# biaslab/GaussianProcessNode

Measured on AMD Instinct MI355X. Metric: VMP iterations/sec (sparse-GP node sweep, kin40k-shaped synthetic), higher is better.
Workload: dtype f64

## Files before the change

gaussianprocessnode_amd/csrc/sgp_api.hip:

```cpp
#include "../../include/sgp_hip.h"
#include "sgp_kernels.hip.h"

#include <algorithm>
#include <atomic>
#include <chrono>
#include <cmath>
#include <cstdio>
#include <cstdlib>
#include <dlfcn.h>
#include <cstring>
#include <limits>
#include <mutex>
#include <string>
#include <type_traits>
#include <vector>

using namespace sgp;

namespace {

thread_local std::string g_create_error;
std::atomic<int> g_live_handles{0};

std::mutex g_registry_mutex;
// ... 276 lines not shown
    SyrkGeom g;
    g.row_lo = row_lo;
    g.nrows = nrows;
    g.tile0 = row_lo * (row_lo + 1) / 2;
    g.ntiles = (row_lo + nrows) * (row_lo + nrows + 1) / 2 - g.tile0;
    g.chunk = wide ? 4 * SYRK_WAVES : KB;
    g.nchunks = 0;
    g.wide = wide ? 1 : 0;
    if (n <= 0) return g;
    if (wide) {
        const int want = std::max(1, std::max(8, cus) / g.ntiles);
        int64_t per = (n + want - 1) / want;
        per = std::max<int64_t>(4 * SYRK_WAVES, (per + 4 * SYRK_WAVES - 1) / (4 * SYRK_WAVES) * (4 * SYRK_WAVES));
        g.chunk = (int)per;
        g.nchunks = (int)std::max<int64_t>(1, (n + per - 1) / per);
        return g;
    }
    const int slots = SYRK_BLOCKS_PER_CU * std::max(8, cus);
    int a = 8;
    for (int q = 2; q <= 8; q *= 2)
        if (g.ntiles % q == 0) a = 8 / q;
    int want = std::max(1, slots / g.ntiles);
    if (want > a) want = want / a * a;
    int64_t per = (n + want - 1) / want;
    per = std::max<int64_t>(KB, (per + KB - 1) / KB * KB);
    g.chunk = (int)per;
    g.nchunks = (int)std::max<int64_t>(1, (n + per - 1) / per);
    if (g.nchunks > a) g.nchunks = (g.nchunks + a - 1) / a * a;
    return g;
}
static inline size_t syrk_items(const SyrkGeom& g) { return (size_t)g.ntiles * g.nchunks; }
static inline unsigned assemble_z(const SyrkGeom& g) { return g.nchunks <= 24 ? 4u : 16u; }
static void launch_syrk(const SyrkGeom& g, hipStream_t s, const double* Kuf, const double* omega, double* slabs, int Mp, int64_t n,
                        int64_t* stamps, long long* gate, long long gate_value) {
    if (g.wide)
        hipLaunchKernelGGL(k_syrk_direct, dim3((unsigned)((syrk_items(g) + 7) / 8 * 8)), dim3(SYRK_DIRECT_THREADS), 0, s, Kuf, omega, slabs, Mp, n,
                           g, stamps, gate, gate_value);
    else
        hipLaunchKernelGGL(k_syrk_stream, dim3((unsigned)syrk_items(g)), dim3(256), 0, s, Kuf, omega, slabs, Mp, n, g, stamps, gate,
                           gate_value);
}

struct PotrfSeq {
    double* A; int ld, Tn; int* info; int n_valid; double* scratch; hipStream_t s;
    double* Winv; LamForm form; bool has_form; double* Sacc; const double* tv_xi; double* tv_t; const hipEvent_t* step_wait;
    int j = 0;
    PotrfSeq(double* A_, int ld_, int Tn_, int* info_, int n_valid_, double* scratch_, hipStream_t s_, double* Winv_ = nullptr,
             const LamForm* form_ = nullptr, double* Sacc_ = nullptr, const double* tv_xi_ = nullptr, double* tv_t_ = nullptr,
             const hipEvent_t* step_wait_ = nullptr)
        : A(A_), ld(ld_), Tn(Tn_), info(info_), n_valid(n_valid_), scratch(scratch_), s(s_), Winv(Winv_), has_form(form_ != nullptr),
          Sacc(Sacc_), tv_xi(tv_xi_), tv_t(tv_t_), step_wait(step_wait_) {
        if (form_) form = *form_;
        else { memset(&form, 0, sizeof form); }
    }
    int extras(int jj) const {
        if (!Winv) return 0;
        int e = 0;
        if (jj >= 2) {
            e += 2 * (jj - 1) * (jj < Tn ? 2 : 1);
            if (Sacc && jj < Tn) e += (jj - 1) * jj / 2;
        }
        if (tv_t && jj >= 1) e += 1;
        return e;
    }
    bool done() const { return j > Tn; }
    void next() {
        LamForm none;
        memset(&none, 0, sizeof none);
        none.trace_chain = has_form ? 1 : 0;
        if (j < Tn) {
            const int nt = Tn - j;
            if (step_wait && step_wait[j]) (void)hipStreamWaitEvent(s, step_wait[j], 0);
            hipLaunchKernelGGL(k_potrf_step, dim3(nt * (nt + 1) / 2 + potrf_twins(Tn, j) + extras(j)), dim3(PSTEP_THREADS), 0, s, A, ld, j, Tn, info,
                               n_valid, scratch, Winv, Sacc, tv_xi, tv_t, has_form ? form : none);
        } else if (j == Tn && Winv && extras(Tn) > 0) {
            hipLaunchKernelGGL(k_potrf_step, dim3(extras(Tn)), dim3(PSTEP_THREADS), 0, s, A, ld, Tn, Tn, info, n_valid, scratch, Winv, Sacc,
                               tv_xi, tv_t, none);
        }
        ++j;
    }
};
static void launch_potrf(double* A, int ld, int Tn, int* info, int n_valid, double* scratch, hipStream_t s,
                         double* Winv = nullptr, const LamForm* form = nullptr, double* Sacc = nullptr,
                         const double* tv_xi = nullptr, double* tv_t = nullptr, const hipEvent_t* step_wait = nullptr) {
    PotrfSeq q(A, ld, Tn, info, n_valid, scratch, s, Winv, form, Sacc, tv_xi, tv_t, step_wait);
    while (!q.done()) q.next();
}

static void launch_ata(const double* W, double* C, int ld, int Tn, hipStream_t s, int rev = 0, const double* mu = nullptr,
                       double* R = nullptr, const double* Psi2 = nullptr, const double* Kinv = nullptr,
                       double* trace_part = nullptr, const UvArgs* uv = nullptr, const double* Sacc = nullptr) {
    const int extra = uv ? Tn * Tn : 0;
    hipLaunchKernelGGL(k_gemm32, dim3(Tn * (Tn + 1) / 2 * 4 + extra), dim3(256), 0, s, W, W, C, ld, Tn, 0, 0, rev, mu, R, Psi2,
                       Kinv, trace_part, uv ? *uv : UvArgs{}, Sacc);
}
static void launch_gemm(const double* A, const double* B, double* C, int ld, int Tn, hipStream_t s) {
    hipLaunchKernelGGL(k_gemm32, dim3(Tn * Tn * 4), dim3(256), 0, s, A, B, C, ld, Tn, 3, 0, 0, (const double*)nullptr, (double*)nullptr,
                       (const double*)nullptr, (const double*)nullptr, (double*)nullptr, UvArgs{}, (const double*)nullptr);
}


extern "C" int sgp_abi_version(void) { return SGP_ABI_VERSION; }

extern "C" const char* sgp_last_error(const sgp_handle* h) { return h ? h->err.c_str() : g_create_error.c_str(); }

template <typename T>
static hipError_t dalloc(T** p, size_t count) {
    *p = nullptr;
    if (count == 0) count = 1;
    return hipMalloc(reinterpret_cast<void**>(p), count * sizeof(T));
}

extern "C" int sgp_create(const sgp_config* cfg, sgp_handle** out) {
    if (!cfg || !out) return fail(nullptr, SGP_ERR_ARG, "sgp_create: null argument");
    *out = nullptr;
    if (cfg->m < 1 || cfg->d < 1 || cfg->d > MAXD || cfg->d_out < 1 || cfg->d_out > MAXO || cfg->n_max < 1)
        return fail(nullptr, SGP_ERR_ARG, "sgp_create: need m >= 1, 1 <= d <= 32, 1 <= d_out <= 4, n_max >= 1");
    if ((int64_t)cfg->m * cfg->d_out > CU_MAXQ - TB)
        return fail(nullptr, SGP_ERR_ARG, "sgp_create: d_out * m is limited to 4032 in this build");
    int ndev = 0;
    if (hipGetDeviceCount(&ndev) != hipSuccess || ndev == 0)
        return fail(nullptr, SGP_ERR_NODEVICE, "sgp_create: no HIP device visible (the HIP path has no CPU fallback)");
    if (cfg->device < 0 || cfg->device >= ndev) return fail(nullptr, SGP_ERR_ARG, "sgp_create: bad device ordinal");
    HIPCHK((sgp_handle*)nullptr, hipSetDevice(cfg->device));
    hipDeviceProp_t prop;
    HIPCHK((sgp_handle*)nullptr, hipGetDeviceProperties(&prop, cfg->device));
    if (strncmp(prop.gcnArchName, "gfx950", 6) != 0)
        return fail(nullptr, SGP_ERR_NODEVICE, "sgp_create: device is not gfx950 (MI355X); this library is built for gfx950 only");
// ... 595 lines not shown
    prep_main(h, s, h->n <= 0);
    if (h->n > 0) {
        launch_gram(h, s, true);
        long long* gate = h->gate_side ? h->dJoin + WORD_GATE : nullptr;
        launch_syrk(h->geom, s, h->dKuf, omega_of(h), h->dSlabs, Mp, h->n, h->dStamps + STAMP_STRIDE * SGP_T_SYRK, gate, h->gate_epoch);
    }
    SyrkGeom ga = h->geom;
    if (h->n <= 0) { ga = syrk_geometry(0, T, h->num_cus, 0); }
    hipLaunchKernelGGL(k_assemble, dim3(T, T + 1, assemble_z(ga)), dim3(256), 0, s, h->dSlabs, h->dBpart, h->dDataScal,
                       pack ? h->dPack : h->dStats, Mp, T, ga, h->n > 0 ? h->nblk : 0, h->dout,
                       SGP_S_COUNT + h->dout * h->dout, 1, h->dStamps + STAMP_STRIDE * SGP_T_LOCAL, h->dInfo + 1, (long long*)nullptr, 0LL,
                       pack ? 1 : 0, h->dBred);
}

static int exchange_stats(sgp_handle* h, hipStream_t s, int tile0, int ntile, bool with_tail);
static int enqueue_stats_overlapped(sgp_handle* h, const SweepPlan& p) {
    const int Mp = h->Mp, T = h->T;
    hipStream_t own = p.stream;
    const bool sharded = p.pack;
    prep_main(h, own, h->n <= 0);
    if (h->n > 0) launch_gram(h, own, true);
    hipLaunchKernelGGL(k_join_wait, dim3(1), dim3(64), 0, h->statM, (const long long*)(h->dJoin + WORD_ASM0), h->stat_epoch,
                       h->spin_limit, h->dInfo + 3, (int)SYNC_LATE_COLUMN, 8);
    for (int g = 0; g < h->ngroups; ++g) {
        const StatGroup& G = h->grp[g];
        hipStream_t s = G.masked ? h->statM : own;
        if (h->n > 0)
            launch_syrk(G.geom, s, h->dKuf, omega_of(h), h->dSlabs + G.slab_off, Mp, h->n,
                        h->dStamps + STAMP_STRIDE * SGP_T_SYRK, g == 0 ? h->dJoin + WORD_GATE : (long long*)nullptr, h->gate_epoch);
        hipLaunchKernelGGL(k_assemble, dim3(G.nrows, T + (g == 0 ? 1 : 0), assemble_z(G.geom)), dim3(256), 0, s, h->dSlabs + G.slab_off, h->dBpart,
                           h->dDataScal, sharded ? h->dPack : h->dStats, Mp, T, G.geom, h->nblk, h->dout,
                           SGP_S_COUNT + h->dout * h->dout, g == 0 ? 1 : 0, h->dStamps + STAMP_STRIDE * SGP_T_LOCAL,
                           g == 0 ? h->dInfo + 1 : (int*)nullptr, g == 0 ? h->dJoin + WORD_ASM0 : (long long*)nullptr, h->stat_epoch,
                           sharded ? 1 : 0, h->dBred);
        if (sharded) {
            if (int xrc = exchange_stats(h, s, G.geom.tile0, G.geom.ntiles, g == 0)) return xrc;
            if (G.masked && hipEventRecord(h->evGroup[g], s) != hipSuccess) return fail(h, SGP_ERR_HIP, "hipEventRecord failed (statistics group)");
        } else if (G.masked)
            hipLaunchKernelGGL(k_join_set, dim3(1), dim3(64), 0, s, h->dJoin + WORD_GROUP0 + g, h->stat_epoch);
    }
    return 0;
}

static void enqueue_finish1(sgp_handle* h, hipStream_t s, const SweepPlan& p) {
    const int M = h->M, Mp = h->Mp, Q = h->Q, Qp = h->Qp, TQ = h->TQ;
    LamForm form;
    memset(&form, 0, sizeof form);
    form.stats = h->dStats; form.Lambda0 = h->dLambda0; form.xi0 = h->dXi0; form.xi = h->dXi; form.P = h->dParams;
    form.M = M; form.Mp = Mp; form.d_out = h->dout; form.Q = Q; form.prior_form = h->prior_form;
    form.stamps = h->dStamps + STAMP_STRIDE * SGP_T_FINISH1;
    form.spin_limit = h->spin_limit;
    form.sync_status = h->dInfo + 3;
    form.trace_chain = 1;
    hipEvent_t step_wait[LAM_MAX_COLS] = {nullptr};
    bool any_wait = false;
    if (p.overlapped) {
        form.col_words = h->dJoin + WORD_GROUP0;
        form.col_need = h->stat_epoch;
        for (int g = 0; g < h->ngroups; ++g) {
            for (int c = h->grp[g].c0; c < h->grp[g].c1; ++c) {
                form.form_step[c] = (unsigned char)h->grp[g].form_step;
                form.col_group[c] = (h->grp[g].masked && !p.pack && !p.resident) ? (unsigned char)g : (unsigned char)0xff;
            }
            if (h->grp[g].masked && p.pack && !p.resident) { step_wait[h->grp[g].form_step] = h->evGroup[g]; any_wait = true; }
        }
    }
    double* uvt0 = h->dUvWork + 2 * (size_t)Qp;
    PotrfSeq lam(h->dLam, Qp, TQ, h->dInfo + 1, Qp, h->dScratch + POTRF_SCRATCH, s, h->dWl, &form, h->dTmp, h->dXi, uvt0,
                 any_wait ? step_wait : nullptr);
    if (p.kuu_interleaved) {
        PotrfSeq kuu(h->dKuu, h->Mp, h->T, h->dInfo + 0, h->M, h->dScratch, h->side, h->dWk, nullptr, h->dSaccK);
        while (!lam.done() || !kuu.done()) {
            if (!lam.done()) lam.next();
            if (!kuu.done()) kuu.next();
        }
        kuu_tail(h, h->side, p.join_word);
    } else {
        while (!lam.done()) lam.next();
    }
    double* uvp = h->dXi;
    double* uvck = h->dUvWork;
    double* uvak = h->dUvWork + Qp;
    double* uvt = uvt0;
    double* uvpart = uvt + (size_t)TQ * Qp;
    hipLaunchKernelGGL(k_trmv_mu_scan, dim3(Qp / 4 + 1 + TQ * (TQ + 1) / 2), dim3(256), 0, s, (const double*)h->dWl,
                       (const double*)uvt, h->dMu, uvp, uvck, uvak, uvpart, Qp);
}

static double* mirror_for(const sgp_handle* h) {
    return (h->hMirror && !h->env_no_zero_copy && !h->training) ? h->hMirror : nullptr;
}

static void launch_traces(sgp_handle* h, hipStream_t s) {
    hipLaunchKernelGGL(k_trace_kinv, dim3(TRACE_BLOCKS), dim3(256), 0, s, h->dStats, h->dKinv, h->dTrace, h->M, h->Mp);
    hipLaunchKernelGGL(k_trace_R, dim3(TRACE_BLOCKS), dim3(256), 0, s, h->dStats, h->dR, h->dTrace + TRACE_BLOCKS, h->M, h->Mp, h->dout,
                       h->Qp, (int64_t*)nullptr);
}

static void enqueue_finish2(sgp_handle* h, hipStream_t s, bool join_word) {
    const int M = h->M, Mp = h->Mp, Q = h->Q, Qp = h->Qp, TQ = h->TQ;
    double* uvp = h->dXi;
    double* uvck = h->dUvWork;
    double* uvak = h->dUvWork + Qp;
    double* uvpart = h->dUvWork + 2 * (size_t)Qp + (size_t)TQ * Qp;
    const int nata = TQ * (TQ + 1) / 2 * 4;
    double* traceR = h->dTrace + TRACE_BLOCKS;
    const double* partK = h->dTrace;
    int nK = TRACE_BLOCKS, nR = TRACE_BLOCKS;
    UvArgs uv;
    uv.Wp = h->dWl; uv.p = uvp; uv.ck = uvck; uv.ak = uvak; uv.partial = uvpart; uv.LR = h->dUvT;
    uv.stamps = h->dStamps + STAMP_STRIDE * SGP_T_FINISH1;
    uv.join = join_word ? h->dJoin + WORD_JOIN : nullptr;
    uv.join_need = h->join_epoch;
    uv.spin_limit = h->spin_limit;
    uv.sync_status = h->dInfo + 3;
    if (h->dout == 1) {
        launch_ata(h->dWl, h->dSigma, Qp, TQ, s, 1, h->dMu, h->dR, h->dStats, h->dKinv, traceR, &uv, h->dTmp);
        partK = traceR + nata;
        nK = nR = nata;
    } else {
        launch_ata(h->dWl, h->dSigma, Qp, TQ, s, 1, h->dMu, h->dR, nullptr, nullptr, nullptr, &uv, h->dTmp);
        launch_traces(h, s);
    }
    hipLaunchKernelGGL(k_scalars, dim3(1), dim3(256), 0, s, h->dStats, partK, nK, (const double*)traceR, nR, h->dMu, h->dKuu,
                       h->dLam, h->dInfo, h->dParams, h->dOut, h->dWishart, M, Mp, h->dout, Q, Qp, Qp - Q,
                       h->dStamps + STAMP_STRIDE * SGP_T_FINISH2, h->dStamps, h->dStampTotals,
                       h->dJoin + WORD_DONE, h->done_epoch,
                       (const double*)(h->dScratch + POTRF_LOGDET), h->T, (const double*)(h->dScratch + POTRF_SCRATCH + POTRF_LOGDET), TQ,
                       mirror_for(h));
}

static int set_device_checked(int device) {
    int ndev = 0;
    if (hipGetDeviceCount(&ndev) != hipSuccess || ndev == 0) return fail(nullptr, SGP_ERR_NODEVICE, "no HIP device visible");
    if (device < 0 || device >= ndev) return fail(nullptr, SGP_ERR_ARG, "bad device ordinal");
    if (hipSetDevice(device) != hipSuccess) return fail(nullptr, SGP_ERR_HIP, "hipSetDevice failed");
    return 0;
}

// ... 1162 lines not shown
```

gaussianprocessnode_amd/csrc/sgp_kernels.hip.h:

```cpp
#pragma once
#include <hip/hip_runtime.h>
#include <stdint.h>
#include <utility>

namespace sgp {

constexpr int TB = 64;
constexpr int PS = 80;
constexpr int KB = 16;
constexpr int MAXD = 32;
constexpr int MAXO = 4;
constexpr int LT = TB + 1;

typedef double d4 __attribute__((ext_vector_type(4)));

struct Params {
    double sigma2;
    double jitter;
    double E_logw;
    double n_override;
    double inv_ell[MAXD];
    double W[MAXO * MAXO];
    double prior_iso;
    double pad[7];
// ... 1144 lines not shown
            acc = __builtin_amdgcn_mfma_f64_16x16x4f64(Wt[(rb + li) * LT + rb + 4 * s4 + lk], Tw[(4 * s4 + lk) * 17 + li],
                                                       acc, 0, 0, 0);
#pragma unroll
        for (int r = 0; r < 4; ++r) Wt[(rb + lk + 4 * r) * LT + cb + li] = -acc[r];
    }
    __syncthreads();
    {
        const int ti = wave >> 1, tj = wave & 1;
        d4 acc = (d4){0.0, 0.0, 0.0, 0.0};
#pragma unroll
        for (int s4 = 0; s4 < 8; ++s4)
            acc = __builtin_amdgcn_mfma_f64_16x16x4f64(S[(32 + 16 * ti + li) * LT + 4 * s4 + lk],
                                                       Wt[(4 * s4 + lk) * LT + 16 * tj + li], acc, 0, 0, 0);
#pragma unroll
        for (int r = 0; r < 4; ++r) T[(16 * ti + lk + 4 * r) * 33 + 16 * tj + li] = acc[r];
        __syncthreads();
        acc = (d4){0.0, 0.0, 0.0, 0.0};
#pragma unroll
        for (int s4 = 0; s4 < 8; ++s4)
            acc = __builtin_amdgcn_mfma_f64_16x16x4f64(Wt[(32 + 16 * ti + li) * LT + 32 + 4 * s4 + lk],
                                                       T[(4 * s4 + lk) * 33 + 16 * tj + li], acc, 0, 0, 0);
#pragma unroll
        for (int r = 0; r < 4; ++r) Wt[(32 + 16 * ti + lk + 4 * r) * LT + 16 * tj + li] = -acc[r];
    }
    __syncthreads();
}

struct TileRegs { double v[16]; };
__device__ __forceinline__ void tile_g2r(TileRegs& t, const double* __restrict__ A, size_t ld, int row0, int col0) {
#pragma unroll
    for (int u = 0; u < 8; ++u) {
        const int e = (threadIdx.x & 255) + 256 * u, c = e >> 5, r = (e & 31) * 2;
        const double2 w = *reinterpret_cast<const double2*>(A + (size_t)(col0 + c) * ld + row0 + r);
        t.v[2 * u] = w.x;
        t.v[2 * u + 1] = w.y;
    }
}
constexpr int LAM_MAX_GROUPS = 8;
constexpr int LAM_MAX_COLS = 64;
struct LamForm {
    const double* stats;
    const double* Lambda0;
    const double* xi0;
    double* xi;
    const Params* P;
    int M, Mp, d_out, Q, prior_form;
    int64_t* stamps;
    const long long* col_words;
    long long col_need;
    unsigned char form_step[LAM_MAX_COLS], col_group[LAM_MAX_COLS];
    int spin_limit;
    int* sync_status;
    int trace_chain;
};
__device__ __forceinline__ double load_agent(const double* p) {
    return __hip_atomic_load((const __attribute__((address_space(1))) double*)p, __ATOMIC_RELAXED, __HIP_MEMORY_SCOPE_AGENT);
}
template <bool DENSE, bool MULTI, bool BYPASS = false>
__device__ __forceinline__ double lambda_entry(const LamForm& f, int gi, int gj, int Qp, double prior_iso, double w00) {
    const bool inside = gi < f.Q && gj < f.Q;
    const int si = inside ? gi : 0, sj = inside ? gj : 0;
    int a = 0, i = si, b = 0, j = sj;
    if constexpr (MULTI) { a = si / f.M; i = si % f.M; b = sj / f.M; j = sj % f.M; }
    double psi;
    if constexpr (BYPASS) psi = load_agent(f.stats + (size_t)j * f.Mp + i); else psi = f.stats[(size_t)j * f.Mp + i];
    const double diag = (gi == gj) ? 1.0 : 0.0;
    double prior, w;
    if constexpr (DENSE) prior = f.Lambda0[(size_t)sj * Qp + si]; else prior = diag * prior_iso;
    if constexpr (MULTI) w = f.P->W[a + b * f.d_out]; else w = w00;
    const double m = inside ? 1.0 : 0.0;
    return fma(m * w, psi, fma(m, prior, (1.0 - m) * diag));
}
template <bool DENSE, bool MULTI, bool BYPASS>
__device__ __forceinline__ void tile_form_r_impl(TileRegs& t, const LamForm& f, int Qp, int row0, int col0) {
    const double prior_iso = BYPASS ? load_agent(&f.P->prior_iso) : f.P->prior_iso, w00 = BYPASS ? load_agent(&f.P->W[0]) : f.P->W[0];
#pragma unroll
    for (int u = 0; u < 16; ++u) {
        const int e = (threadIdx.x & 255) + 256 * (u >> 1), c = e >> 5, r = (e & 31) * 2 + (u & 1);
        t.v[u] = lambda_entry<DENSE, MULTI, BYPASS>(f, Qp - 1 - (row0 + r), Qp - 1 - (col0 + c), Qp, prior_iso, w00);
    }
}
__device__ __forceinline__ void tile_form_r(TileRegs& t, const LamForm& f, int Qp, int row0, int col0, bool bypass = false) {
    const bool dense = f.prior_form == 1, multi = f.d_out > 1;
    if (bypass && !multi) {
        if (dense) tile_form_r_impl<true, false, true>(t, f, Qp, row0, col0); else tile_form_r_impl<false, false, true>(t, f, Qp, row0, col0);
        return;
    }
    if (dense) { if (multi) tile_form_r_impl<true, true, false>(t, f, Qp, row0, col0); else tile_form_r_impl<true, false, false>(t, f, Qp, row0, col0); }
    else       { if (multi) tile_form_r_impl<false, true, false>(t, f, Qp, row0, col0); else tile_form_r_impl<false, false, false>(t, f, Qp, row0, col0); }
}
__device__ __forceinline__ void tile_r2s(double* S, const TileRegs& t) {
#pragma unroll
    for (int u = 0; u < 16; ++u) {
        const int e = (threadIdx.x & 255) + 256 * (u >> 1), c = e >> 5, r = (e & 31) * 2 + (u & 1);
        S[r * LT + c] = t.v[u];
    }
}
__device__ __forceinline__ void tile_g2s(double* S, const double* __restrict__ A, size_t ld, int row0, int col0) {
    TileRegs t;
    tile_g2r(t, A, ld, row0, col0);
    tile_r2s(S, t);
}
__device__ __forceinline__ void tile_fetch(TileRegs& t, bool do_form, bool load_old, const double* __restrict__ A, const LamForm& f,
                                           int ld, int row0, int col0, bool bypass) {
    if (do_form) {
        tile_form_r(t, f, ld, row0, col0, bypass);
// ... 211 lines not shown
            const int row = wave * 16 + lk + 4 * r;
            Bs[row * PS32 + li] = t0a[r] + t0b[r];
            Bs[row * PS32 + 16 + li] = t1a[r] + t1b[r];
        }
        __syncthreads();
        d4 o0a = Z, o1a = Z, o0b = Z, o1b = Z;
        winv_half_mma(o0a, o1a, o0b, o1b, As, Bs, lane, wave);
        __syncthreads();
#pragma unroll
        for (int r = 0; r < 4; ++r) { o0[r] = -(o0a[r] + o0b[r]); o1[r] = -(o1a[r] + o1b[r]); }
    }
#pragma unroll
    for (int r = 0; r < 4; ++r) {
        const int row = wave * 16 + lk + 4 * r;
        Os[li * LT + row] = o0[r];
        Os[(16 + li) * LT + row] = o1[r];
    }
    __syncthreads();
    for (int e = tid; e < 32 * TB; e += 256) {
        const int jj = e >> 6, r = e & 63;
        W[(size_t)(col0 + jj) * ld + i * TB + r] = Os[jj * LT + r];
    }
}

__device__ __forceinline__ void sigma_row_tile(const double* __restrict__ W, double* __restrict__ Sacc, int ld, int i, int I,
                                               int J, double* panels, double* tile) {
    const int tid = threadIdx.x, lane = tid & 63, wave = tid >> 6, wr = wave >> 1, wc = wave & 1;
    double* As = panels;
    double* Bs = panels + TB * PS;
    load_panel_t(As, W, ld, i * TB, I * TB, TB, tid);
    if (I != J) load_panel_t(Bs, W, ld, i * TB, J * TB, TB, tid);
    if (I == i) {
        for (int e = tid; e < TB * LT; e += 256) tile[e] = 0.0;
    } else {
        tile_g2s(tile, Sacc, ld, I * TB, J * TB);
    }
    __syncthreads();
    Acc4 acc;
    acc_zero(acc);
    tile_mma(acc, As, (I != J) ? Bs : As, TB, lane, wr, wc);
#pragma unroll
    for (int ti = 0; ti < 2; ++ti)
#pragma unroll
        for (int tj = 0; tj < 2; ++tj)
#pragma unroll
            for (int r = 0; r < 4; ++r) acc.t[ti][tj][r] = -acc.t[ti][tj][r];
    tile_sub_acc(tile, acc, lane, wr, wc);
    __syncthreads();
    tile_s2g(tile, Sacc, ld, I * TB, J * TB);
}

template <int NP>
__device__ __forceinline__ void tvec_role(const double* __restrict__ L, const double* __restrict__ W,
                                          const double* __restrict__ xi, double* __restrict__ t, int ld, int i, double* lds) {
    constexpr int CP = TB / NP;
    double* red = lds;
    double* rvec = lds + NP * TB;
    const int tid = threadIdx.x, r = tid & 63, part = tid >> 6;
    const double* wb = W + (size_t)(i * TB + CP * part) * ld + i * TB + r;
    double wv[CP];
#pragma unroll
    for (int u = 0; u < CP; ++u) wv[u] = wb[(size_t)u * ld];
    double acc = 0.0;
    for (int k = 0; k < i; k += 4) {
        double v[4][CP], tv[4][CP];
#pragma unroll
        for (int q = 0; q < 4; ++q) {
            const int kq = (k + q < i) ? k + q : i - 1;
            const double live = (k + q < i) ? 1.0 : 0.0;
            const double* base = L + (size_t)(kq * TB + CP * part) * ld + i * TB + r;
#pragma unroll
            for (int u = 0; u < CP; ++u) { v[q][u] = base[(size_t)u * ld]; tv[q][u] = t[kq * TB + CP * part + u] * live; }
        }
#pragma unroll
        for (int q = 0; q < 4; ++q)
#pragma unroll
            for (int u = 0; u < CP; ++u) acc = fma(v[q][u], tv[q][u], acc);
    }
    auto tree = [&](int row) {
        double a[NP];
#pragma unroll
        for (int q = 0; q < NP; ++q) a[q] = red[q * TB + row];
#pragma unroll
        for (int w = 1; w < NP; w <<= 1)
#pragma unroll
            for (int q = 0; q + w < NP; q += 2 * w) a[q] += a[q + w];
        return a[0];
    };
    red[part * TB + r] = acc;
    __syncthreads();
    if (part == 0) rvec[r] = xi[ld - 1 - (i * TB + r)] - tree(r);
    __syncthreads();
    double s = 0.0;
#pragma unroll
    for (int u = 0; u < CP; ++u) s = fma(wv[u], rvec[CP * part + u], s);
    __syncthreads();
    red[part * TB + r] = s;
    __syncthreads();
    if (part == 0) t[i * TB + r] = tree(r);
}

__device__ __forceinline__ void form_xi(const LamForm& form, int ld, int tid, bool bypass = false) {
    const double* B = form.stats + (size_t)form.Mp * form.Mp;
    for (int gi = tid; gi < ld; gi += 256) {
        double v = 0.0;
        if (gi < form.Q) {
            const int aa = gi / form.M, i = gi % form.M;
            v = (form.prior_form == 1) ? form.xi0[gi] : 0.0;
            for (int e = 0; e < form.d_out; ++e) {
                const double* bp = B + (size_t)e * form.Mp + i;
                const double* wp = &form.P->W[e + aa * form.d_out];
                v = fma(bypass ? load_agent(bp) : *bp, bypass ? load_agent(wp) : *wp, v);
            }
        }
        form.xi[gi] = v;
    }
}
__device__ __forceinline__ bool wait_stat_group(const LamForm& f, int g) {
    int late = 0;
    if ((threadIdx.x & 63) == 0) {
        const long long* w = f.col_words + g;
        if (!join_ready(w, f.col_need)) {
            late = 1;
            spin_until(w, f.col_need, f.spin_limit, f.sync_status, SYNC_LATE_COLUMN);
        }
    }
    return __builtin_amdgcn_readfirstlane(late) != 0;
}

__device__ long long g_step_trace[8 * 64];
#ifndef SGP_STEP_TRACE_A
#define SGP_STEP_TRACE_A 1
#endif
#ifdef SGP_STEP_TRACE
#define STEP_TRACE(e) do { if (tv_t && a == SGP_STEP_TRACE_A && b == 0 && tw == 0 && lane == 0 && wave == 0 && j < 8) g_step_trace[j * 64 + (xgroup ? 32 : 0) + (e)] = realtime_ticks(); } while (0)
#else
#define STEP_TRACE(e) do { } while (0)
#endif

constexpr int PSTEP_THREADS = 512;
constexpr int POTRF_TWINS = 2;
__host__ __device__ constexpr int potrf_twins(int Tn, int j) { return (Tn - j >= 2) ? POTRF_TWINS : 0; }
constexpr int POTRF_SCRATCH = 3 * TB * TB + 64 + 64;
constexpr int POTRF_LOGDET = 3 * TB * TB + 64;
__global__ void __launch_bounds__(PSTEP_THREADS) k_potrf_step(double* __restrict__ A, int ld, int j, int Tn, int* __restrict__ info,
                                                    int n_valid, double* __restrict__ scratch, double* __restrict__ Winv,
                                                    double* __restrict__ Sacc, const double* __restrict__ tv_xi,
                                                    double* __restrict__ tv_t, LamForm form) {
    __shared__ __attribute__((aligned(16))) double lds[2 * TB * PS];
    __shared__ __attribute__((aligned(16))) double tiles[2 * TB * LT];
    __shared__ double dprep[4 * DPB];
    __shared__ double rinv[TB];
    TraceScope trace((form.trace_chain ? 16 : 40) + j);
    const bool xgroup = threadIdx.x >= 256;
    const int tid = threadIdx.x & 255, lane = tid & 63, wave = tid >> 6, wr = wave >> 1, wc = wave & 1;
    {
        const int npot = (Tn - j) * (Tn - j + 1) / 2 + potrf_twins(Tn, j);
        if ((int)blockIdx.x >= npot) {
            int e = blockIdx.x - npot;
            const int nfin = (j >= 2) ? 2 * (j - 1) : 0;
            const int npre = (j < Tn) ? nfin : 0;
            const int nsig = (Sacc && j >= 2 && j < Tn) ? (j - 1) * j / 2 : 0;
            if (e >= nfin + npre + nsig) { tvec_role<8>(A, Winv, tv_xi, tv_t, ld, j - 1, lds); return; }
            if (xgroup) return;
            if (e < nfin) winv_row_tile(A, Winv, ld, j - 1, e >> 1, e & 1, lds, 2, tiles);
            else if (e < nfin + npre) { e -= nfin; winv_row_tile(A, Winv, ld, j, e >> 1, e & 1, lds, 1); }
            else if (e < nfin + npre + nsig) {
                int I, J;
                tile_from_index(e - nfin - npre, I, J);
                sigma_row_tile(Winv, Sacc, ld, j - 2, I, J, lds, tiles);
            }
            return;
        }
    }
    int a, b, tw = 0;
    {
        const int nown = (Tn - j) * (Tn - j + 1) / 2;
        if ((int)blockIdx.x >= nown) { a = 1; b = 0; tw = blockIdx.x - nown + 1; }
        else tile_from_index(blockIdx.x, a, b);
    }
    const int i0 = (j + a) * TB, k0 = (j + b) * TB, j0 = j * TB;
    double* P0 = lds;
    double* P1 = lds + TB * PS;
    double* S = tiles;
    double* X = tiles + TB * LT;
    Acc4 accX;
    acc_zero(accX);
    const bool panel = (b == 0);
    const bool diag_inv = panel && a == 0 && Winv != nullptr;
    if (xgroup && !(panel && (a != 0 || diag_inv))) return;
    const bool lam = form.stats != nullptr;
    const int fstep = lam ? (int)form.form_step[j + b] : -1;
    const bool do_form = lam && fstep == j;
    const bool load_old = !lam || fstep < j || j >= 2;
    const bool xi_duty = lam && j == 0 && blockIdx.x == gridDim.x - 1;
    if (!lam && j == 0 && !panel) return;
    bool bypass = false;
    if (lam && form.col_words) {
        if (xi_duty && form.col_group[0] != 0xff) bypass = wait_stat_group(form, form.col_group[0]);
        if (do_form && form.col_group[j + b] != 0xff) bypass = wait_stat_group(form, form.col_group[j + b]) || bypass;
        if (j == 0 && !do_form) {
            if (xi_duty) form_xi(form, ld, tid, bypass);
            return;
        }
        if (blockIdx.x == 0 && !xgroup) trace_mark(200 + j);
    }
    double* Dn_out = scratch + (size_t)(1 + (j & 1)) * TB * TB;
    const double* Dn_in = scratch + (size_t)(2 - (j & 1)) * TB * TB;
    auto move_prev = [&]() {
        const int q0 = (j - 1) * TB;
        for (int e = tid; e < TB * TB; e += 256) A[(size_t)(q0 + (e >> 6)) * ld + q0 + (e & 63)] = scratch[e];
    };
    TileRegs rX, rS, rD;
    if (lam && j == 0) stamp_enter(form.stamps);
    STEP_TRACE(0);
    if (panel) {
// ... 304 lines not shown
            if (Psi2) {
                tsum = fma(rv[0], p0.x, fma(rv[1], p0.y, fma(rv[2], p1.x, rv[3] * p1.y)));
                if (kinv_late) {
                    if (spin_until(uv.join, uv.join_need, uv.spin_limit, uv.sync_status, SYNC_LATE_KINV)) {
                        const __attribute__((address_space(1))) double* kq = (const __attribute__((address_space(1))) double*)(Kinv + offA);
                        q0.x = __hip_atomic_load(kq + 0, __ATOMIC_RELAXED, __HIP_MEMORY_SCOPE_AGENT);
                        q0.y = __hip_atomic_load(kq + 1, __ATOMIC_RELAXED, __HIP_MEMORY_SCOPE_AGENT);
                        q1.x = __hip_atomic_load(kq + 2, __ATOMIC_RELAXED, __HIP_MEMORY_SCOPE_AGENT);
                        q1.y = __hip_atomic_load(kq + 3, __ATOMIC_RELAXED, __HIP_MEMORY_SCOPE_AGENT);
                    } else
                        q0.x = __builtin_nan("");
                }
                tsumK = fma(q0.x, p0.x, fma(q0.y, p0.y, fma(q1.x, p1.x, q1.y * p1.y)));
            }
        }
    }
    {
        double v[4];
#pragma unroll
        for (int e = 0; e < 4; ++e) v[e] = Qd[(o4 + (rev ? 3 - e : e)) * 33 + oc];
        *reinterpret_cast<double2*>(C + offB) = make_double2(v[0], v[1]);
        *reinterpret_cast<double2*>(C + offB + 2) = make_double2(v[2], v[3]);
        if (mu) {
            double rv[4];
#pragma unroll
            for (int e = 0; e < 4; ++e) rv[e] = fma(muB[e], muB[4], v[e]);
            *reinterpret_cast<double2*>(R + offB) = make_double2(rv[0], rv[1]);
            *reinterpret_cast<double2*>(R + offB + 2) = make_double2(rv[2], rv[3]);
        }
    }
    if (trace_part) {
        if (I != J) { tsum *= 2.0; tsumK *= 2.0; }
        tsum = block_sum(tsum, tred);
        tsumK = block_sum(tsumK, tred);
        if (tid == 0) {
            trace_part[blockIdx.x] = tsum;
            trace_part[Tn * (Tn + 1) / 2 * 4 + blockIdx.x] = tsumK;
        }
    }
}

__global__ void __launch_bounds__(256) k_symv(const double* __restrict__ S, const double* __restrict__ x,
                                              double* __restrict__ y, int n, int ld) {
    const int row = blockIdx.x * 4 + (threadIdx.x >> 6), lane = threadIdx.x & 63;
    if (row >= n) return;
    double s = 0.0;
    for (int j = lane; j < n; j += 64) s = fma(S[(size_t)row * ld + j], x[j], s);
    for (int o = 32; o > 0; o >>= 1) s += __shfl_xor(s, o);
    if (lane == 0) y[row] = s;
}

constexpr int CU_MAXQ = 4096;

__global__ void __launch_bounds__(256) k_trmv_mu_scan(const double* __restrict__ W, const double* __restrict__ tpart ,
                                                      double* __restrict__ mu, double* __restrict__ p,
                                                      double* __restrict__ ck, double* __restrict__ ak,
                                                      double* __restrict__ uvpart, int Qp) {
    __shared__ double ts[CU_MAXQ];
    TraceScope trace(4);
    const int lane = threadIdx.x & 63;
    const bool matvec = (int)blockIdx.x < Qp / 4;
    const int kcol = blockIdx.x * 4 + (threadIdx.x >> 6);
    double wv[8] = {0.0, 0.0, 0.0, 0.0, 0.0, 0.0, 0.0, 0.0};
    if (matvec) {
        const double* col = W + (size_t)kcol * Qp;
#pragma unroll
        for (int u = 0; u < 8; ++u) {
            const int i = kcol + lane + 64 * u;
            wv[u] = col[min(i, Qp - 1)] * ((i < Qp) ? 1.0 : 0.0);
        }
    }
    for (int i = threadIdx.x; i < Qp; i += 256) ts[i] = tpart[i];
    __syncthreads();
    if ((int)blockIdx.x > Qp / 4) {
        if (threadIdx.x >= 64) return;
        int jb, kb;
        tile_from_index(blockIdx.x - Qp / 4 - 1, jb, kb);
        const int j = 64 * jb + lane;
        double v[64];
        load_v_column(v, W, Qp, kb, j);
        double sacc = 0.0;
#pragma unroll
        for (int kk = 0; kk < 64; ++kk) sacc = fma(ts[Qp - 1 - (64 * kb + kk)], v[kk], sacc);
        uvpart[(size_t)kb * Qp + j] = sacc;
        return;
    }
    if ((int)blockIdx.x == Qp / 4) {
        if (threadIdx.x >= 64) return;
        const int per = (Qp + 63) / 64;
        const int e0 = lane * per, e1 = min((lane + 1) * per, Qp);
        double loc = 0.0;
        for (int e = e0; e < e1; ++e) { double v = ts[Qp - 1 - e]; p[e] = v; loc = fma(v, v, loc); }
        double inc = loc;
        for (int o = 1; o < 64; o <<= 1) {
            double u = __shfl_up(inc, o);
            if (lane >= o) inc += u;
        }
        double alpha = 1.0 + (inc - loc);
        for (int e = e0; e < e1; ++e) {
            const double pe = ts[Qp - 1 - e], an = fma(pe, pe, alpha);
            const double ir = 1.0 / sqrt(alpha * an);
            ck[e] = an * ir;
            ak[e] = pe * ir;
            alpha = an;
        }
        return;
    }
    const int k = kcol;
    const double* col = W + (size_t)k * Qp;
    double s = 0.0;
#pragma unroll
    for (int u = 0; u < 8; ++u) s = fma(wv[u], ts[min(k + lane + 64 * u, Qp - 1)], s);
    for (int i = k + lane + 512; i < Qp; i += 64) s = fma(col[i], ts[i], s);
    for (int o = 32; o > 0; o >>= 1) s += __shfl_xor(s, o);
    if (lane == 0) mu[Qp - 1 - k] = s;
}

constexpr int TRACE_BLOCKS = 64;
constexpr int TRACE_SLOTS = 1 + MAXO * MAXO;


__global__ void __launch_bounds__(256) k_trace_kinv(const double* __restrict__ stats, const double* __restrict__ Kinv,
                                                    double* __restrict__ partial, int M, int Mp) {
    __shared__ double red[4];
    const double* Psi2 = stats;
    const int tid = threadIdx.x;
    double t1 = 0.0;
    for (int j = blockIdx.x; j < M; j += gridDim.x)
        for (int i = tid; i < M; i += 256) t1 = fma(Kinv[(size_t)j * Mp + i], Psi2[(size_t)j * Mp + i], t1);
    t1 = block_sum(t1, red);
    if (tid == 0) partial[blockIdx.x] = t1;
}

__global__ void __launch_bounds__(256) k_trace_R(const double* __restrict__ stats, const double* __restrict__ R,
                                                 double* __restrict__ partial, int M, int Mp, int d_out, int Qp,
                                                 int64_t* stamps) {
    __shared__ double red[4];
    stamp_enter(stamps);
    const double* Psi2 = stats;
    const int tid = threadIdx.x;
    for (int a = 0; a < d_out; ++a)
        for (int b = 0; b < d_out; ++b) {
            double t2 = 0.0;
            for (int j = blockIdx.x; j < M; j += gridDim.x)
                for (int i = tid; i < M; i += 256)
                    t2 = fma(R[(size_t)(b * M + j) * Qp + a * M + i], Psi2[(size_t)j * Mp + i], t2);
            t2 = block_sum(t2, red);
            if (tid == 0) partial[(size_t)blockIdx.x * d_out * d_out + a + b * d_out] = t2;
        }
}

__global__ void __launch_bounds__(256) k_scalars(const double* __restrict__ stats, const double* __restrict__ partK, int nK,
                                                 const double* __restrict__ partR, int nR,
                                                 const double* __restrict__ mu, const double* __restrict__ Lkuu,
                                                 const double* __restrict__ Llam, const int* __restrict__ info,
                                                 const Params* __restrict__ P, double* __restrict__ out,
                                                 double* __restrict__ wishart, int M, int Mp, int d_out, int Q, int Qp,
                                                 int lam_off, int64_t* stamps, int64_t* all_stamps,
                                                 int64_t* totals, long long* done_word, long long done_value,
                                                 const double* __restrict__ ldK, int nldK, const double* __restrict__ ldL, int nldL,
                                                 double* __restrict__ mirror) {
    __shared__ double red[4];
    __shared__ double redn[4 * 5];
    __shared__ double tr[TRACE_SLOTS];
    TraceScope trace(7);
    stamp_enter(stamps);
    const double* B = stats + (size_t)Mp * Mp;
// ... 869 lines not shown
```

Before: 4633.

## Merge final potrf tail step into trmv/mu scan kernel

The last tvec block parks its residual in scratch. The separate tail k_potrf_step launch that finished the Winv rows and the t vector for the final tile is dropped, and that work is folded into k_trmv_mu_scan. Each block now recomputes the last-tile W·residual product in LDS, and the matvec blocks also fix up their own last-tile W entries, removing one serialized kernel launch from the latency-bound Cholesky chain. In exchange every trmv block does redundant small matvecs, uses more dynamic LDS and takes extra syncthreads. The change also carries correctness risk in the in-place W update and in the uv blocks that skip kb==0.

```diff
diff --git a/gaussianprocessnode_amd/csrc/sgp_api.hip b/gaussianprocessnode_amd/csrc/sgp_api.hip
--- a/gaussianprocessnode_amd/csrc/sgp_api.hip
+++ b/gaussianprocessnode_amd/csrc/sgp_api.hip
@@ -352,7 +352,10 @@
           Sacc(Sacc_), tv_xi(tv_xi_), tv_t(tv_t_), step_wait(step_wait_) {
         if (form_) form = *form_;
         else { memset(&form, 0, sizeof form); }
-    }
+        if (!(Winv && tv_t && Tn >= 2)) form.tail_merged = 0;
+    }
+    bool tail_merged() const { return form.tail_merged != 0; }
+    const double* resid() const { return tail_merged() ? scratch + POTRF_RESID : nullptr; }
     int extras(int jj) const {
         if (!Winv) return 0;
         int e = 0;
@@ -363,7 +366,7 @@
         if (tv_t && jj >= 1) e += 1;
         return e;
     }
-    bool done() const { return j > Tn; }
+    bool done() const { return j > Tn - (tail_merged() ? 1 : 0); }
     void next() {
         LamForm none;
         memset(&none, 0, sizeof none);
@@ -373,7 +376,7 @@
             if (step_wait && step_wait[j]) (void)hipStreamWaitEvent(s, step_wait[j], 0);
             hipLaunchKernelGGL(k_potrf_step, dim3(nt * (nt + 1) / 2 + potrf_twins(Tn, j) + extras(j)), dim3(PSTEP_THREADS), 0, s, A, ld, j, Tn, info,
                                n_valid, scratch, Winv, Sacc, tv_xi, tv_t, has_form ? form : none);
-        } else if (j == Tn && Winv && extras(Tn) > 0) {
+        } else if (j == Tn && Winv && extras(Tn) > 0 && !tail_merged()) {
             hipLaunchKernelGGL(k_potrf_step, dim3(extras(Tn)), dim3(PSTEP_THREADS), 0, s, A, ld, Tn, Tn, info, n_valid, scratch, Winv, Sacc,
                                tv_xi, tv_t, none);
         }
@@ -1075,6 +1078,7 @@
     form.spin_limit = h->spin_limit;
     form.sync_status = h->dInfo + 3;
     form.trace_chain = 1;
+    form.tail_merged = 1;
     hipEvent_t step_wait[LAM_MAX_COLS] = {nullptr};
     bool any_wait = false;
     if (p.overlapped) {
@@ -1106,8 +1110,9 @@
     double* uvak = h->dUvWork + Qp;
     double* uvt = uvt0;
     double* uvpart = uvt + (size_t)TQ * Qp;
-    hipLaunchKernelGGL(k_trmv_mu_scan, dim3(Qp / 4 + 1 + TQ * (TQ + 1) / 2), dim3(256), 0, s, (const double*)h->dWl,
-                       (const double*)uvt, h->dMu, uvp, uvck, uvak, uvpart, Qp);
+    const size_t trmv_lds = sizeof(double) * ((size_t)Qp + (lam.resid() ? TRMV_FIN_LDS : 0));
+    hipLaunchKernelGGL(k_trmv_mu_scan, dim3(Qp / 4 + 1 + TQ * (TQ + 1) / 2), dim3(256), trmv_lds, s, h->dWl, (const double*)h->dLam,
+                       lam.resid(), uvt, h->dMu, uvp, uvck, uvak, uvpart, Qp);
 }
 
 static double* mirror_for(const sgp_handle* h) {
diff --git a/gaussianprocessnode_amd/csrc/sgp_kernels.hip.h b/gaussianprocessnode_amd/csrc/sgp_kernels.hip.h
--- a/gaussianprocessnode_amd/csrc/sgp_kernels.hip.h
+++ b/gaussianprocessnode_amd/csrc/sgp_kernels.hip.h
@@ -1220,6 +1220,7 @@
     int spin_limit;
     int* sync_status;
     int trace_chain;
+    int tail_merged;
 };
 __device__ __forceinline__ double load_agent(const double* p) {
     return __hip_atomic_load((const __attribute__((address_space(1))) double*)p, __ATOMIC_RELAXED, __HIP_MEMORY_SCOPE_AGENT);
@@ -1537,7 +1538,8 @@
 
 template <int NP>
 __device__ __forceinline__ void tvec_role(const double* __restrict__ L, const double* __restrict__ W,
-                                          const double* __restrict__ xi, double* __restrict__ t, int ld, int i, double* lds) {
+                                          const double* __restrict__ xi, double* __restrict__ t, int ld, int i, double* lds,
+                                          double* __restrict__ park = nullptr) {
     constexpr int CP = TB / NP;
     double* red = lds;
     double* rvec = lds + NP * TB;
@@ -1546,22 +1548,6 @@
     double wv[CP];
 #pragma unroll
     for (int u = 0; u < CP; ++u) wv[u] = wb[(size_t)u * ld];
-    double acc = 0.0;
-    for (int k = 0; k < i; k += 4) {
-        double v[4][CP], tv[4][CP];
-#pragma unroll
-        for (int q = 0; q < 4; ++q) {
-            const int kq = (k + q < i) ? k + q : i - 1;
-            const double live = (k + q < i) ? 1.0 : 0.0;
-            const double* base = L + (size_t)(kq * TB + CP * part) * ld + i * TB + r;
-#pragma unroll
-            for (int u = 0; u < CP; ++u) { v[q][u] = base[(size_t)u * ld]; tv[q][u] = t[kq * TB + CP * part + u] * live; }
-        }
-#pragma unroll
-        for (int q = 0; q < 4; ++q)
-#pragma unroll
-            for (int u = 0; u < CP; ++u) acc = fma(v[q][u], tv[q][u], acc);
-    }
     auto tree = [&](int row) {
         double a[NP];
 #pragma unroll
@@ -1572,17 +1558,42 @@
             for (int q = 0; q + w < NP; q += 2 * w) a[q] += a[q + w];
         return a[0];
     };
-    red[part * TB + r] = acc;
-    __syncthreads();
-    if (part == 0) rvec[r] = xi[ld - 1 - (i * TB + r)] - tree(r);
-    __syncthreads();
-    double s = 0.0;
-#pragma unroll
-    for (int u = 0; u < CP; ++u) s = fma(wv[u], rvec[CP * part + u], s);
-    __syncthreads();
-    red[part * TB + r] = s;
-    __syncthreads();
-    if (part == 0) t[i * TB + r] = tree(r);
+#pragma unroll 1
+    for (int b = i;; ++b) {
+        double acc = 0.0;
+        for (int k = 0; k < b; k += 4) {
+            double v[4][CP], tv[4][CP];
+#pragma unroll
+            for (int q = 0; q < 4; ++q) {
+                const int kq = (k + q < b) ? k + q : b - 1;
+                const double live = (k + q < b) ? 1.0 : 0.0;
+                const double* base = L + (size_t)(kq * TB + CP * part) * ld + b * TB + r;
+#pragma unroll
+                for (int u = 0; u < CP; ++u) { v[q][u] = base[(size_t)u * ld]; tv[q][u] = t[kq * TB + CP * part + u] * live; }
+            }
+#pragma unroll
+            for (int q = 0; q < 4; ++q)
+#pragma unroll
+                for (int u = 0; u < CP; ++u) acc = fma(v[q][u], tv[q][u], acc);
+        }
+        red[part * TB + r] = acc;
+        __syncthreads();
+        if (part == 0) rvec[r] = xi[ld - 1 - (b * TB + r)] - tree(r);
+        __syncthreads();
+        if (b != i) {
+            if (part == 0) park[r] = rvec[r];
+            return;
+        }
+        double s = 0.0;
+#pragma unroll
+        for (int u = 0; u < CP; ++u) s = fma(wv[u], rvec[CP * part + u], s);
+        __syncthreads();
+        red[part * TB + r] = s;
+        __syncthreads();
+        if (part == 0) t[i * TB + r] = tree(r);
+        if (!park) return;
+        __syncthreads();
+    }
 }
 
 __device__ __forceinline__ void form_xi(const LamForm& form, int ld, int tid, bool bypass = false) {
@@ -1626,8 +1637,9 @@
 constexpr int PSTEP_THREADS = 512;
 constexpr int POTRF_TWINS = 2;
 __host__ __device__ constexpr int potrf_twins(int Tn, int j) { return (Tn - j >= 2) ? POTRF_TWINS : 0; }
-constexpr int POTRF_SCRATCH = 3 * TB * TB + 64 + 64;
+constexpr int POTRF_SCRATCH = 3 * TB * TB + 64 + 64 + 64;
 constexpr int POTRF_LOGDET = 3 * TB * TB + 64;
+constexpr int POTRF_RESID = 3 * TB * TB + 128;
 __global__ void __launch_bounds__(PSTEP_THREADS) k_potrf_step(double* __restrict__ A, int ld, int j, int Tn, int* __restrict__ info,
                                                     int n_valid, double* __restrict__ scratch, double* __restrict__ Winv,
                                                     double* __restrict__ Sacc, const double* __restrict__ tv_xi,
@@ -1646,7 +1658,10 @@
             const int nfin = (j >= 2) ? 2 * (j - 1) : 0;
             const int npre = (j < Tn) ? nfin : 0;
             const int nsig = (Sacc && j >= 2 && j < Tn) ? (j - 1) * j / 2 : 0;
-            if (e >= nfin + npre + nsig) { tvec_role<8>(A, Winv, tv_xi, tv_t, ld, j - 1, lds); return; }
+            if (e >= nfin + npre + nsig) {
+                tvec_role<8>(A, Winv, tv_xi, tv_t, ld, j - 1, lds, (form.tail_merged && j == Tn - 1) ? scratch + POTRF_RESID : nullptr);
+                return;
+            }
             if (xgroup) return;
             if (e < nfin) winv_row_tile(A, Winv, ld, j - 1, e >> 1, e & 1, lds, 2, tiles);
             else if (e < nfin + npre) { e -= nfin; winv_row_tile(A, Winv, ld, j, e >> 1, e & 1, lds, 1); }
@@ -2057,30 +2072,41 @@
 
 constexpr int CU_MAXQ = 4096;
 
-__global__ void __launch_bounds__(256) k_trmv_mu_scan(const double* __restrict__ W, const double* __restrict__ tpart ,
+constexpr int TRMV_FIN_LDS = TB * TB / 2 + 4 * TB;
+__global__ void __launch_bounds__(256) k_trmv_mu_scan(double* __restrict__ W, const double* __restrict__ L,
+                                                      const double* __restrict__ resid, double* __restrict__ tpart ,
                                                       double* __restrict__ mu, double* __restrict__ p,
                                                       double* __restrict__ ck, double* __restrict__ ak,
                                                       double* __restrict__ uvpart, int Qp) {
-    __shared__ double ts[CU_MAXQ];
+    extern __shared__ __attribute__((aligned(16))) double trmv_lds[];
+    double* ts = trmv_lds;
     TraceScope trace(4);
-    const int lane = threadIdx.x & 63;
+    const int lane = threadIdx.x & 63, wave = threadIdx.x >> 6;
+    const bool fin = resid != nullptr;
+    const int i0 = Qp - TB;
+    const int lim = fin ? i0 : Qp;
     const bool matvec = (int)blockIdx.x < Qp / 4;
-    const int kcol = blockIdx.x * 4 + (threadIdx.x >> 6);
+    const int kcol = blockIdx.x * 4 + wave;
     double wv[8] = {0.0, 0.0, 0.0, 0.0, 0.0, 0.0, 0.0, 0.0};
     if (matvec) {
         const double* col = W + (size_t)kcol * Qp;
 #pragma unroll
         for (int u = 0; u < 8; ++u) {
             const int i = kcol + lane + 64 * u;
-            wv[u] = col[min(i, Qp - 1)] * ((i < Qp) ? 1.0 : 0.0);
-        }
-    }
-    for (int i = threadIdx.x; i < Qp; i += 256) ts[i] = tpart[i];
-    __syncthreads();
+            const double w = col[min(i, Qp - 1)];
+            wv[u] = (i < lim) ? w : 0.0;
+        }
+    }
+    auto copy_t = [&]() {
+        for (int i = threadIdx.x; i < lim; i += 256) ts[i] = tpart[i];
+    };
     if ((int)blockIdx.x > Qp / 4) {
-        if (threadIdx.x >= 64) return;
         int jb, kb;
         tile_from_index(blockIdx.x - Qp / 4 - 1, jb, kb);
+        if (kb == 0) return;
+        copy_t();
+        __syncthreads();
+        if (threadIdx.x >= 64) return;
         const int j = 64 * jb + lane;
         double v[64];
         load_v_column(v, W, Qp, kb, j);
@@ -2089,6 +2115,68 @@
         for (int kk = 0; kk < 64; ++kk) sacc = fma(ts[Qp - 1 - (64 * kb + kk)], v[kk], sacc);
         uvpart[(size_t)kb * Qp + j] = sacc;
         return;
+    }
+    const bool colfin = fin && matvec && kcol < i0;
+    double tl = 0.0, wl = 0.0;
+    if (fin) {
+        double* Ms = ts + Qp;
+        double* vs = Ms + TB * TB / 2;
+        double* rs = ts + i0;
+        double2 mL[8], mW[8];
+#pragma unroll
+        for (int u = 0; u < 8; ++u) {
+            const int e = threadIdx.x + 256 * u, kk = e >> 5, r = (e & 31) * 2;
+            mW[u] = *reinterpret_cast<const double2*>(W + (size_t)(i0 + kk) * Qp + i0 + r);
+            mL[u] = colfin ? *reinterpret_cast<const double2*>(L + (size_t)(i0 - TB + kk) * Qp + i0 + r) : make_double2(0.0, 0.0);
+        }
+        double a = 0.0, v = 0.0;
+        if (matvec) {
+            const double* col = W + (size_t)kcol * Qp;
+            wl = col[i0 + lane];
+            if (colfin) { v = col[i0 - TB + lane]; a = (kcol < i0 - TB) ? wl : 0.0; }
+        }
+        const double rv = resid[lane];
+        copy_t();
+        if (wave == 0) rs[lane] = rv;
+        if (colfin) vs[wave * TB + lane] = v;
+        auto stage = [&](const double2 (&m)[8], int half) {
+#pragma unroll
+            for (int u = 0; u < 4; ++u) *reinterpret_cast<double2*>(Ms + 2 * (threadIdx.x + 256 * u)) = m[4 * half + u];
+            __syncthreads();
+        };
+        auto half_matvec = [&](double (&c)[4], const double* x, int half, int k0, int n) {
+#pragma unroll 4
+            for (int kk = k0; kk < k0 + n; kk += 4)
+#pragma unroll
+                for (int q = 0; q < 4; ++q) c[q] = fma(Ms[(kk + q) * TB + lane], x[32 * half + kk + q], c[q]);
+        };
+        double c[4] = {0.0, 0.0, 0.0, 0.0};
+        if (colfin) {
+            stage(mL, 0);
+            half_matvec(c, vs + wave * TB, 0, 0, 32);
+            __syncthreads();
+            stage(mL, 1);
+            half_matvec(c, vs + wave * TB, 1, 0, 32);
+            a += (c[0] + c[1]) + (c[2] + c[3]);
+            vs[wave * TB + lane] = a;
+            __syncthreads();
+        }
+        double d[4] = {0.0, 0.0, 0.0, 0.0};
+        c[0] = c[1] = c[2] = c[3] = 0.0;
+        stage(mW, 0);
+        if (colfin) half_matvec(c, vs + wave * TB, 0, 0, 32);
+        half_matvec(d, rs, 0, 8 * wave, 8);
+        __syncthreads();
+        stage(mW, 1);
+        if (colfin) { half_matvec(c, vs + wave * TB, 1, 0, 32); wl = -((c[0] + c[1]) + (c[2] + c[3])); }
+        half_matvec(d, rs, 1, 8 * wave, 8);
+        vs[wave * TB + lane] = (d[0] + d[1]) + (d[2] + d[3]);
+        __syncthreads();
+        tl = (vs[lane] + vs[TB + lane]) + (vs[2 * TB + lane] + vs[3 * TB + lane]);
+        if (!matvec && wave == 0) { ts[i0 + lane] = tl; tpart[i0 + lane] = tl; }
+    } else {
+        copy_t();
+        __syncthreads();
     }
     if ((int)blockIdx.x == Qp / 4) {
         if (threadIdx.x >= 64) return;
@@ -2112,12 +2200,18 @@
         return;
     }
     const int k = kcol;
-    const double* col = W + (size_t)k * Qp;
+    double* col = W + (size_t)k * Qp;
+    if (colfin) col[i0 + lane] = wl;
     double s = 0.0;
 #pragma unroll
-    for (int u = 0; u < 8; ++u) s = fma(wv[u], ts[min(k + lane + 64 * u, Qp - 1)], s);
-    for (int i = k + lane + 512; i < Qp; i += 64) s = fma(col[i], ts[i], s);
+    for (int u = 0; u < 8; ++u) s = fma(wv[u], ts[min(k + lane + 64 * u, lim - 1)], s);
+    for (int i = k + lane + 512; i < lim; i += 64) s = fma(col[i], ts[i], s);
     for (int o = 32; o > 0; o >>= 1) s += __shfl_xor(s, o);
+    if (fin) {
+        double sl = wl * tl;
+        for (int o = 32; o > 0; o >>= 1) sl += __shfl_xor(sl, o);
+        s += sl;
+    }
     if (lane == 0) mu[Qp - 1 - k] = s;
 }
 
```

Result: no change. 4611 (-0.5%).
